# SimonZeng7108/efficientsam3

Measured on NVIDIA H100. Metric: encoder images/sec @1024^2 (EV-M student forward), higher is better.
Workload: dtype bf16

## Files before the change

### efficientsam3_b200/csrc/litemla_tc.cu

```cuda
#include "ptx.cuh"

namespace es3 {
namespace {
__device__ __forceinline__ void ldsm4t(uint32_t addr, uint32_t& r0, uint32_t& r1, uint32_t& r2, uint32_t& r3) {
  asm volatile("ldmatrix.sync.aligned.m8n8.x4.trans.shared.b16 {%0,%1,%2,%3}, [%4];"
               : "=r"(r0), "=r"(r1), "=r"(r2), "=r"(r3) : "r"(addr));
}
__device__ __forceinline__ void cpa16(uint32_t saddr, const void* g, bool valid) {
  const int sz = valid ? 16 : 0;
  asm volatile("cp.async.cg.shared.global [%0], [%1], 16, %2;" ::"r"(saddr), "l"(g), "r"(sz) : "memory");
}
__device__ __forceinline__ void cpa_wait_all() { asm volatile("cp.async.commit_group;\ncp.async.wait_group 0;" ::: "memory"); }
__device__ __forceinline__ uint32_t relu_bf16x2(uint32_t v) {
  uint32_t r;
  asm("max.bf16x2 %0, %1, %2;" : "=r"(r) : "r"(v), "r"(0u));
  return r;
}
}

constexpr int AG_TH = 16, AG_TW = 32, AG_IH = AG_TH + 4, AG_IW = AG_TW + 4, AG_PS = 48;
constexpr int AG_TILE_BYTES = AG_IH * AG_IW * AG_PS;

constexpr int AG2_SMEM = AG_TILE_BYTES + 25 * 16 * 2 + 16 * AG_PS;
__global__ void __launch_bounds__(256, 3) litemla_aggreg_dwpw_kernel(const bf16* ms_in, bf16* ms_out, long long ld,
                                                                  const bf16* __restrict__ wdw, const bf16* __restrict__ wpw,
                                                                  int H, int W, int tiles_x) {
  extern __shared__ __align__(16) uint8_t smem[];
  const uint32_t u_tile = static_cast<uint32_t>(__cvta_generic_to_shared(smem));
  const bf16* s_wd = reinterpret_cast<const bf16*>(smem + AG_TILE_BYTES);
  const uint32_t u_wp = u_tile + AG_TILE_BYTES + 25 * 16 * 2;
  const int tid = threadIdx.x, warp = tid >> 5, lane = tid & 31;
  const int tile = blockIdx.x, grp = blockIdx.y, b = blockIdx.z;
  const int oy0 = (tile / tiles_x) * AG_TH, ox0 = (tile % tiles_x) * AG_TW;

  const bf16* xb = ms_in + (long long)b * H * W * ld + grp * 16;
  for (int i = tid; i < AG_IH * AG_IW * 2; i += 256) {
    const int v = i & 1, p = i >> 1;
    const int iy = oy0 - 2 + p / AG_IW, ix = ox0 - 2 + p % AG_IW;
    const bool ok = iy >= 0 && iy < H && ix >= 0 && ix < W;
    cpa16(u_tile + p * AG_PS + v * 16, ok ? xb + ((long long)iy * W + ix) * ld + v * 8 : xb, ok);
  }
  if (tid < 50) cpa16(u_tile + AG_TILE_BYTES + tid * 16, wdw + (long long)grp * 400 + tid * 8, true);
  if (tid >= 64 && tid < 96) {
    const int i = tid - 64, n = i >> 1, v = i & 1;
    cpa16(u_wp + n * AG_PS + v * 16, wpw + ((long long)grp * 16 + n) * 16 + v * 8, true);
  }
  cpa_wait_all();
  __syncthreads();

  const int a_row = lane & 15, a_kh = lane >> 4;
  const int b_n = (lane & 7) + ((lane >> 4) << 3), b_kh = (lane >> 3) & 1;
  const int g = lane >> 2, t4 = lane & 3;
  const uint32_t dshift = (g & 1) ? 16u : 0u;
  const bool dvalid = (g >> 1) == t4;
  float acc[4][2][4];
#pragma unroll
  for (int m = 0; m < 4; ++m)
#pragma unroll
    for (int n = 0; n < 2; ++n) { acc[m][n][0] = acc[m][n][1] = acc[m][n][2] = acc[m][n][3] = 0.f; }

  const int xh = warp & 1, y0 = (warp >> 1) * 4;
#pragma unroll 1
  for (int kx = 0; kx < 5; ++kx) {
    uint32_t af[8][4];
#pragma unroll
    for (int r = 0; r < 8; ++r)
      ptx::ldsm_x4(u_tile + ((y0 + r) * AG_IW + xh * 16 + a_row + kx) * AG_PS + a_kh * 16, af[r][0], af[r][1], af[r][2], af[r][3]);
    uint32_t b_lo[5], b_hi[5];
#pragma unroll
    for (int ky = 0; ky < 5; ++ky) {
      const uint32_t w_lo = (uint32_t)__bfloat16_as_ushort(s_wd[(ky * 5 + kx) * 16 + g]);
      const uint32_t w_hi = (uint32_t)__bfloat16_as_ushort(s_wd[(ky * 5 + kx) * 16 + 8 + g]);
      b_lo[ky] = dvalid ? (w_lo << dshift) : 0u;
      b_hi[ky] = dvalid ? (w_hi << dshift) : 0u;
    }
#pragma unroll
    for (int m = 0; m < 4; ++m) {
#pragma unroll
      for (int kp = 0; kp < 2; ++kp) {
        const uint32_t a_lo[4] = {af[m + 2 * kp][0], af[m + 2 * kp][1], af[m + 2 * kp + 1][0], af[m + 2 * kp + 1][1]};
        const uint32_t a_hi[4] = {af[m + 2 * kp][2], af[m + 2 * kp][3], af[m + 2 * kp + 1][2], af[m + 2 * kp + 1][3]};
        ptx::mma_16816(acc[m][0], a_lo, b_lo[2 * kp], b_lo[2 * kp + 1]);
        ptx::mma_16816(acc[m][1], a_hi, b_hi[2 * kp], b_hi[2 * kp + 1]);
      }
      ptx::mma_1688(acc[m][0], af[m + 4][0], af[m + 4][1], b_lo[4]);
      ptx::mma_1688(acc[m][1], af[m + 4][2], af[m + 4][3], b_hi[4]);
    }
  }
  uint32_t p0, p1, p2, p3;
  ptx::ldsm_x4(u_wp + b_n * AG_PS + b_kh * 16, p0, p1, p2, p3);
  bf16* ob = ms_out + (long long)b * H * W * ld + grp * 16;
#pragma unroll
  for (int m = 0; m < 4; ++m) {
    const uint32_t pa[4] = {pack_bf16x2(acc[m][0][0], acc[m][0][1]), pack_bf16x2(acc[m][0][2], acc[m][0][3]),
                            pack_bf16x2(acc[m][1][0], acc[m][1][1]), pack_bf16x2(acc[m][1][2], acc[m][1][3])};
    float o[2][4] = {{0.f, 0.f, 0.f, 0.f}, {0.f, 0.f, 0.f, 0.f}};
    ptx::mma_16816(o[0], pa, p0, p1);
    ptx::mma_16816(o[1], pa, p2, p3);
    const int oy = oy0 + y0 + m;
    if (oy >= H) continue;
#pragma unroll
    for (int half = 0; half < 2; ++half) {
      const int ox = ox0 + xh * 16 + g + half * 8;
      if (ox >= W) continue;
      bf16* dst = ob + ((long long)oy * W + ox) * ld + t4 * 2;
      *reinterpret_cast<uint32_t*>(dst) = pack_bf16x2(o[0][half * 2], o[0][half * 2 + 1]);
      *reinterpret_cast<uint32_t*>(dst + 8) = pack_bf16x2(o[1][half * 2], o[1][half * 2 + 1]);
    }
  }
}

constexpr int KV_PX = 512, KV_RS = 80;

__global__ void __launch_bounds__(256) litemla_kv_tc_kernel(const bf16* __restrict__ ms, long long ld,
                                                            float* __restrict__ part, int HW) {
  __shared__ __align__(16) uint8_t s_kv[KV_PX * KV_RS];
  const uint32_t u = static_cast<uint32_t>(__cvta_generic_to_shared(s_kv));
  const int tid = threadIdx.x, warp = tid >> 5, lane = tid & 31;
  const int h = blockIdx.y, b = blockIdx.z, heads2 = gridDim.y, nchunk = gridDim.x;
  const int p_base = blockIdx.x * KV_PX;
  const bf16* src = ms + (long long)b * HW * ld + h * 48 + 16;
  for (int i = tid; i < KV_PX * 4; i += 256) {
    const int v = i & 3, pl = i >> 2;
    const bool ok = p_base + pl < HW;
    cpa16(u + pl * KV_RS + v * 16, ok ? src + (long long)(p_base + pl) * ld + v * 8 : src, ok);
  }
  cpa_wait_all();
  __syncthreads();

  const int g = lane >> 2, t4 = lane & 3;
  float acc[2][4], ones[2][4];
#pragma unroll
  for (int n = 0; n < 2; ++n) {
    acc[n][0] = acc[n][1] = acc[n][2] = acc[n][3] = 0.f;
    ones[n][0] = ones[n][1] = ones[n][2] = ones[n][3] = 0.f;
  }
  const uint32_t one2 = (g == 0) ? 0x3F803F80u : 0u;
  const uint32_t a_ones[4] = {one2, 0u, one2, 0u};
  const int av_p = (lane & 7) + ((lane >> 4) << 3), av_c = 32 + ((lane >> 3) & 1) * 16;
  const int bk_p = (lane & 7) + (((lane >> 3) & 1) << 3), bk_c = (lane >> 4) * 16;
#pragma unroll
  for (int ks = 0; ks < 4; ++ks) {
    const int p0 = warp * 64 + ks * 16;
    uint32_t af[4], b0, b1, b2, b3;
    ldsm4t(u + (p0 + av_p) * KV_RS + av_c, af[0], af[1], af[2], af[3]);
    ldsm4t(u + (p0 + bk_p) * KV_RS + bk_c, b0, b1, b2, b3);
    b0 = relu_bf16x2(b0); b1 = relu_bf16x2(b1); b2 = relu_bf16x2(b2); b3 = relu_bf16x2(b3);
    ptx::mma_16816(acc[0], af, b0, b1);
    ptx::mma_16816(acc[1], af, b2, b3);
    ptx::mma_16816(ones[0], a_ones, b0, b1);
    ptx::mma_16816(ones[1], a_ones, b2, b3);
  }
  __syncthreads();
  float* red = reinterpret_cast<float*>(s_kv);
  float* mine = red + warp * 17 * 16;
#pragma unroll
  for (int n = 0; n < 2; ++n) {
    const int j = n * 8 + t4 * 2;
    mine[g * 16 + j] = acc[n][0];
    mine[g * 16 + j + 1] = acc[n][1];
    mine[(g + 8) * 16 + j] = acc[n][2];
    mine[(g + 8) * 16 + j + 1] = acc[n][3];
    if (g == 0) {
      mine[16 * 16 + j] = ones[n][0];
      mine[16 * 16 + j + 1] = ones[n][1];
    }
  }
  __syncthreads();
  float* dst = part + (((long long)b * heads2 + h) * nchunk + blockIdx.x) * 17 * 16;
  for (int i = tid; i < 17 * 16; i += 256) {
    float s = 0.f;
#pragma unroll
    for (int w = 0; w < 8; ++w) s += red[w * 17 * 16 + i];
    dst[i] = s;
  }
}

__global__ void __launch_bounds__(128) litemla_apply_tc_kernel(const bf16* __restrict__ ms, long long ld,
                                                               const float* __restrict__ part, int nchunk,
                                                               bf16* __restrict__ att, long long ldo, int HW, float eps) {
  __shared__ float skv[17 * 16];
  const int tid = threadIdx.x, warp = tid >> 5, lane = tid & 31;
  const int h = blockIdx.y, b = blockIdx.z, heads2 = gridDim.y;
  const float* src = part + ((long long)b * heads2 + h) * nchunk * 17 * 16;
  for (int i = tid; i < 17 * 16; i += 128) {
    float a = 0.f;
    for (int c = 0; c < nchunk; ++c) a += src[c * 17 * 16 + i];
    skv[i] = a;
  }
  __syncthreads();
  const int g = lane >> 2, t4 = lane & 3;
  uint32_t bh[3][2], bl[3][2];
#pragma unroll
  for (int nt = 0; nt < 3; ++nt) {
    const int d = nt * 8 + g;
#pragma unroll
    for (int kh = 0; kh < 2; ++kh) {
      float v0 = 0.f, v1 = 0.f;
      if (d <= 16) { v0 = skv[d * 16 + kh * 8 + t4 * 2]; v1 = skv[d * 16 + kh * 8 + t4 * 2 + 1]; }
      const uint32_t hi = pack_bf16x2(v0, v1);
      const float2 hf = unpack_bf16x2(hi);
      bh[nt][kh] = hi;
      bl[nt][kh] = pack_bf16x2(v0 - hf.x, v1 - hf.y);
    }
  }
  const bf16* qb = ms + (long long)b * HW * ld + h * 48;
  bf16* ob = att + (long long)b * HW * ldo + h * 16;
#pragma unroll 1
  for (int mt = 0; mt < 4; ++mt) {
    const int p0 = blockIdx.x * 256 + warp * 64 + mt * 16;
    if (p0 >= HW) break;
    const int pa = p0 + g, pb = p0 + g + 8;
    uint32_t af[4] = {0u, 0u, 0u, 0u};
    if (pa < HW) {
      const uint32_t* q = reinterpret_cast<const uint32_t*>(qb + (long long)pa * ld);
      af[0] = relu_bf16x2(__ldg(q + t4));
      af[2] = relu_bf16x2(__ldg(q + 4 + t4));
    }
    if (pb < HW) {
      const uint32_t* q = reinterpret_cast<const uint32_t*>(qb + (long long)pb * ld);
      af[1] = relu_bf16x2(__ldg(q + t4));
      af[3] = relu_bf16x2(__ldg(q + 4 + t4));
    }
    float acc[3][4];
#pragma unroll
    for (int nt = 0; nt < 3; ++nt) {
      acc[nt][0] = acc[nt][1] = acc[nt][2] = acc[nt][3] = 0.f;
      ptx::mma_16816(acc[nt], af, bl[nt][0], bl[nt][1]);
      ptx::mma_16816(acc[nt], af, bh[nt][0], bh[nt][1]);
    }
    const float den_a = __shfl_sync(0xffffffffu, acc[2][0], g * 4);
    const float den_b = __shfl_sync(0xffffffffu, acc[2][2], g * 4);
    const float ia = 1.f / (den_a + eps), ib = 1.f / (den_b + eps);
    if (pa < HW) {
      uint32_t* o = reinterpret_cast<uint32_t*>(ob + (long long)pa * ldo);
      o[t4] = pack_bf16x2(acc[0][0] * ia, acc[0][1] * ia);
      o[4 + t4] = pack_bf16x2(acc[1][0] * ia, acc[1][1] * ia);
    }
    if (pb < HW) {
      uint32_t* o = reinterpret_cast<uint32_t*>(ob + (long long)pb * ldo);
      o[t4] = pack_bf16x2(acc[0][2] * ib, acc[0][3] * ib);
      o[4 + t4] = pack_bf16x2(acc[1][2] * ib, acc[1][3] * ib);
    }
  }
}

}

using namespace es3;

extern "C" int es3_litemla_aggreg_dwpw(void* ms, long long ld, const void* wdw, const void* wpw, int B, int H, int W, int C3,
                                       void* stream) {
  ES3_REQUIRE(C3 % 16 == 0 && ld % 8 == 0 && ld >= 2 * C3, "es3_litemla_aggreg_dwpw: bad C3=%d ld=%lld", C3, ld);
  static bool configured = false;
  if (!configured) {
    ES3_CHECK_CUDA(cudaFuncSetAttribute(litemla_aggreg_dwpw_kernel, cudaFuncAttributeMaxDynamicSharedMemorySize, AG2_SMEM));
    configured = true;
  }
  const int tiles_x = ceil_div(W, AG_TW), tiles_y = ceil_div(H, AG_TH);
  dim3 grid(tiles_x * tiles_y, C3 / 16, B);
  litemla_aggreg_dwpw_kernel<<<grid, 256, AG2_SMEM, (cudaStream_t)stream>>>((const bf16*)ms, (bf16*)ms + C3, ld, (const bf16*)wdw,
                                                                            (const bf16*)wpw, H, W, tiles_x);
  ES3_LAUNCH_CHECK("litemla_aggreg_dwpw_kernel");
  return 0;
}

extern "C" long long es3_litemla_ws_floats(int B, int HW, int heads2) {
  return (long long)B * heads2 * ceil_div(HW, KV_PX) * 17 * 16;
}

extern "C" int es3_litemla_attn_tc(const void* ms, long long ld, float* kv_ws, void* att, long long ldo, int B, int HW,
                                   int heads2, float eps, void* stream) {
  ES3_REQUIRE(ld >= 48 * heads2 && ld % 8 == 0 && ldo % 8 == 0, "es3_litemla_attn_tc: bad ld=%lld ldo=%lld heads2=%d", ld, ldo, heads2);
  cudaStream_t st = (cudaStream_t)stream;
  const int nchunk = ceil_div(HW, KV_PX);
  litemla_kv_tc_kernel<<<dim3(nchunk, heads2, B), 256, 0, st>>>((const bf16*)ms, ld, kv_ws, HW);
  ES3_LAUNCH_CHECK("litemla_kv_tc_kernel");
  litemla_apply_tc_kernel<<<dim3(ceil_div(HW, 256), heads2, B), 128, 0, st>>>((const bf16*)ms, ld, kv_ws, nchunk,
                                                                             (bf16*)att, ldo, HW, eps);
  ES3_LAUNCH_CHECK("litemla_apply_tc_kernel");
  return 0;
}
```

Measured before the change: 4031.

## Make LiteMLA kv/apply kernels persistent, multi-head, cp.async-pipelined, and reverse batch order

The kv and apply attention kernels become persistent-style, sized from SM occupancy. Each CTA handles several heads and several pixel chunks and streams them through a 3-stage cp.async ring, which hides load latency and cuts launch/tail overhead. The apply kernel now stages Q in shared memory and writes outputs through shared memory as coalesced 128-bit stores. The aggreg and apply kernels also walk the batch index in reverse, likely so they reuse the L2-resident data the previous kernel just touched. In exchange, dynamic shared memory and register use grow, and there is extra per-item synchronisation.

New measurement: 4074, median of 6. 1.1% higher.

```diff
diff --git a/efficientsam3_b200/csrc/litemla_tc.cu b/efficientsam3_b200/csrc/litemla_tc.cu
--- a/efficientsam3_b200/csrc/litemla_tc.cu
+++ b/efficientsam3_b200/csrc/litemla_tc.cu
@@ -11,10 +11,29 @@
   asm volatile("cp.async.cg.shared.global [%0], [%1], 16, %2;" ::"r"(saddr), "l"(g), "r"(sz) : "memory");
 }
 __device__ __forceinline__ void cpa_wait_all() { asm volatile("cp.async.commit_group;\ncp.async.wait_group 0;" ::: "memory"); }
+__device__ __forceinline__ void cpa_commit() { asm volatile("cp.async.commit_group;" ::: "memory"); }
+template <int N>
+__device__ __forceinline__ void cpa_wait() { asm volatile("cp.async.wait_group %0;" ::"n"(N) : "memory"); }
 __device__ __forceinline__ uint32_t relu_bf16x2(uint32_t v) {
   uint32_t r;
   asm("max.bf16x2 %0, %1, %2;" : "=r"(r) : "r"(v), "r"(0u));
   return r;
+}
+__device__ __forceinline__ void sts32(uint32_t addr, uint32_t v) { asm volatile("st.shared.b32 [%0], %1;" ::"r"(addr), "r"(v) : "memory"); }
+__device__ __forceinline__ uint4 lds128(uint32_t addr) {
+  uint4 v;
+  asm volatile("ld.shared.v4.b32 {%0,%1,%2,%3}, [%4];" : "=r"(v.x), "=r"(v.y), "=r"(v.z), "=r"(v.w) : "r"(addr) : "memory");
+  return v;
+}
+
+int sm_count() {
+  static int n = 0;
+  if (n == 0) {
+    int dev = 0;
+    ES3_CHECK_CUDA(cudaGetDevice(&dev));
+    ES3_CHECK_CUDA(cudaDeviceGetAttribute(&n, cudaDevAttrMultiProcessorCount, dev));
+  }
+  return n;
 }
 }
 
@@ -30,7 +49,7 @@
   const bf16* s_wd = reinterpret_cast<const bf16*>(smem + AG_TILE_BYTES);
   const uint32_t u_wp = u_tile + AG_TILE_BYTES + 25 * 16 * 2;
   const int tid = threadIdx.x, warp = tid >> 5, lane = tid & 31;
-  const int tile = blockIdx.x, grp = blockIdx.y, b = blockIdx.z;
+  const int tile = blockIdx.x, grp = blockIdx.y, b = gridDim.z - 1 - blockIdx.z;
   const int oy0 = (tile / tiles_x) * AG_TH, ox0 = (tile % tiles_x) * AG_TW;
 
   const bf16* xb = ms_in + (long long)b * H * W * ld + grp * 16;
@@ -110,139 +129,218 @@
   }
 }
 
-constexpr int KV_PX = 512, KV_RS = 80;
-
-__global__ void __launch_bounds__(256) litemla_kv_tc_kernel(const bf16* __restrict__ ms, long long ld,
-                                                            float* __restrict__ part, int HW) {
-  __shared__ __align__(16) uint8_t s_kv[KV_PX * KV_RS];
-  const uint32_t u = static_cast<uint32_t>(__cvta_generic_to_shared(s_kv));
+constexpr int KV_PX = 512, KV_NH = 2, KV_NS = 3;
+constexpr int KV_SPX = 128;
+constexpr int KV_RS = KV_NH * 96 + 16;
+constexpr int KV_STAGE = KV_SPX * KV_RS;
+constexpr int KV_SMEM = KV_NS * KV_STAGE + 8 * KV_NH * 17 * 16 * 4;
+
+__global__ void __launch_bounds__(256, 2) litemla_kv_tc_kernel(const bf16* __restrict__ ms, long long ld,
+                                                               float* __restrict__ part, int HW, int heads2, int nchunk, int cpc) {
+  extern __shared__ __align__(16) uint8_t smem[];
+  const uint32_t u = static_cast<uint32_t>(__cvta_generic_to_shared(smem));
+  float* red = reinterpret_cast<float*>(smem + KV_NS * KV_STAGE);
   const int tid = threadIdx.x, warp = tid >> 5, lane = tid & 31;
-  const int h = blockIdx.y, b = blockIdx.z, heads2 = gridDim.y, nchunk = gridDim.x;
-  const int p_base = blockIdx.x * KV_PX;
-  const bf16* src = ms + (long long)b * HW * ld + h * 48 + 16;
-  for (int i = tid; i < KV_PX * 4; i += 256) {
-    const int v = i & 3, pl = i >> 2;
-    const bool ok = p_base + pl < HW;
-    cpa16(u + pl * KV_RS + v * 16, ok ? src + (long long)(p_base + pl) * ld + v * 8 : src, ok);
-  }
-  cpa_wait_all();
-  __syncthreads();
+  const int h0 = blockIdx.y * KV_NH, b = blockIdx.z, nh = min(KV_NH, heads2 - h0);
+  const int c0 = blockIdx.x * cpc, nc = min(cpc, nchunk - c0), nitems = nc * 4;
+  const bf16* src = ms + (long long)b * HW * ld + h0 * 48;
+
+  auto load_item = [&](int k) {
+    const uint32_t us = u + (k % KV_NS) * KV_STAGE;
+    const int pbase = (c0 + (k >> 2)) * KV_PX + (k & 3) * 16;
+    for (int i = tid; i < KV_SPX * 6 * KV_NH; i += 256) {
+      const int c = i % (6 * KV_NH), r = i / (6 * KV_NH);
+      if (c >= 6 * nh || c % 6 < 2) continue;
+      const int p = pbase + (r >> 4) * 64 + (r & 15);
+      const bool ok = p < HW;
+      cpa16(us + r * KV_RS + c * 16, ok ? src + (long long)p * ld + c * 8 : src, ok);
+    }
+  };
+#pragma unroll
+  for (int s = 0; s < KV_NS - 1; ++s) {
+    if (s < nitems) load_item(s);
+    cpa_commit();
+  }
 
   const int g = lane >> 2, t4 = lane & 3;
-  float acc[2][4], ones[2][4];
-#pragma unroll
-  for (int n = 0; n < 2; ++n) {
-    acc[n][0] = acc[n][1] = acc[n][2] = acc[n][3] = 0.f;
-    ones[n][0] = ones[n][1] = ones[n][2] = ones[n][3] = 0.f;
-  }
   const uint32_t one2 = (g == 0) ? 0x3F803F80u : 0u;
   const uint32_t a_ones[4] = {one2, 0u, one2, 0u};
-  const int av_p = (lane & 7) + ((lane >> 4) << 3), av_c = 32 + ((lane >> 3) & 1) * 16;
-  const int bk_p = (lane & 7) + (((lane >> 3) & 1) << 3), bk_c = (lane >> 4) * 16;
-#pragma unroll
-  for (int ks = 0; ks < 4; ++ks) {
-    const int p0 = warp * 64 + ks * 16;
-    uint32_t af[4], b0, b1, b2, b3;
-    ldsm4t(u + (p0 + av_p) * KV_RS + av_c, af[0], af[1], af[2], af[3]);
-    ldsm4t(u + (p0 + bk_p) * KV_RS + bk_c, b0, b1, b2, b3);
-    b0 = relu_bf16x2(b0); b1 = relu_bf16x2(b1); b2 = relu_bf16x2(b2); b3 = relu_bf16x2(b3);
-    ptx::mma_16816(acc[0], af, b0, b1);
-    ptx::mma_16816(acc[1], af, b2, b3);
-    ptx::mma_16816(ones[0], a_ones, b0, b1);
-    ptx::mma_16816(ones[1], a_ones, b2, b3);
-  }
-  __syncthreads();
-  float* red = reinterpret_cast<float*>(s_kv);
-  float* mine = red + warp * 17 * 16;
-#pragma unroll
-  for (int n = 0; n < 2; ++n) {
-    const int j = n * 8 + t4 * 2;
-    mine[g * 16 + j] = acc[n][0];
-    mine[g * 16 + j + 1] = acc[n][1];
-    mine[(g + 8) * 16 + j] = acc[n][2];
-    mine[(g + 8) * 16 + j + 1] = acc[n][3];
-    if (g == 0) {
-      mine[16 * 16 + j] = ones[n][0];
-      mine[16 * 16 + j + 1] = ones[n][1];
-    }
-  }
-  __syncthreads();
-  float* dst = part + (((long long)b * heads2 + h) * nchunk + blockIdx.x) * 17 * 16;
-  for (int i = tid; i < 17 * 16; i += 256) {
-    float s = 0.f;
-#pragma unroll
-    for (int w = 0; w < 8; ++w) s += red[w * 17 * 16 + i];
-    dst[i] = s;
-  }
-}
-
-__global__ void __launch_bounds__(128) litemla_apply_tc_kernel(const bf16* __restrict__ ms, long long ld,
-                                                               const float* __restrict__ part, int nchunk,
-                                                               bf16* __restrict__ att, long long ldo, int HW, float eps) {
-  __shared__ float skv[17 * 16];
+  const int av_p = (lane & 7) + ((lane >> 4) << 3), av_c = 64 + ((lane >> 3) & 1) * 16;
+  const int bk_p = (lane & 7) + (((lane >> 3) & 1) << 3), bk_c = 32 + (lane >> 4) * 16;
+  float acc[KV_NH][2][4], ones[KV_NH][2][4];
+
+#pragma unroll 1
+  for (int k = 0; k < nitems; ++k) {
+    cpa_wait<KV_NS - 2>();
+    __syncthreads();
+    if (k + KV_NS - 1 < nitems) load_item(k + KV_NS - 1);
+    cpa_commit();
+    const int ks = k & 3;
+    if (ks == 0) {
+#pragma unroll
+      for (int j = 0; j < KV_NH; ++j)
+#pragma unroll
+        for (int n = 0; n < 2; ++n) {
+          acc[j][n][0] = acc[j][n][1] = acc[j][n][2] = acc[j][n][3] = 0.f;
+          ones[j][n][0] = ones[j][n][1] = ones[j][n][2] = ones[j][n][3] = 0.f;
+        }
+    }
+    const uint32_t us = u + (k % KV_NS) * KV_STAGE + warp * 16 * KV_RS;
+#pragma unroll
+    for (int j = 0; j < KV_NH; ++j) {
+      if (j >= nh) break;
+      uint32_t af[4], b0, b1, b2, b3;
+      ldsm4t(us + av_p * KV_RS + j * 96 + av_c, af[0], af[1], af[2], af[3]);
+      ldsm4t(us + bk_p * KV_RS + j * 96 + bk_c, b0, b1, b2, b3);
+      b0 = relu_bf16x2(b0); b1 = relu_bf16x2(b1); b2 = relu_bf16x2(b2); b3 = relu_bf16x2(b3);
+      ptx::mma_16816(acc[j][0], af, b0, b1);
+      ptx::mma_16816(acc[j][1], af, b2, b3);
+      ptx::mma_16816(ones[j][0], a_ones, b0, b1);
+      ptx::mma_16816(ones[j][1], a_ones, b2, b3);
+    }
+    if (ks != 3) continue;
+#pragma unroll
+    for (int j = 0; j < KV_NH; ++j) {
+      float* mine = red + (warp * KV_NH + j) * 17 * 16;
+#pragma unroll
+      for (int n = 0; n < 2; ++n) {
+        const int jj = n * 8 + t4 * 2;
+        mine[g * 16 + jj] = acc[j][n][0];
+        mine[g * 16 + jj + 1] = acc[j][n][1];
+        mine[(g + 8) * 16 + jj] = acc[j][n][2];
+        mine[(g + 8) * 16 + jj + 1] = acc[j][n][3];
+        if (g == 0) {
+          mine[16 * 16 + jj] = ones[j][n][0];
+          mine[16 * 16 + jj + 1] = ones[j][n][1];
+        }
+      }
+    }
+    __syncthreads();
+    const int chunk = c0 + (k >> 2);
+    for (int i = tid; i < nh * 17 * 16; i += 256) {
+      const int j = i / (17 * 16), e = i % (17 * 16);
+      float s = 0.f;
+#pragma unroll
+      for (int w = 0; w < 8; ++w) s += red[(w * KV_NH + j) * 17 * 16 + e];
+      part[(((long long)b * heads2 + h0 + j) * nchunk + chunk) * 17 * 16 + e] = s;
+    }
+  }
+  cpa_wait<0>();
+}
+
+constexpr int AP_NH = 4, AP_NS = 3;
+constexpr int AP_PX = 128;
+constexpr int AP_RS = AP_NH * 32 + 16;
+constexpr int AP_STAGE = AP_PX * AP_RS;
+constexpr int AP_SMEM = AP_NS * AP_STAGE + AP_NH * 17 * 16 * 4;
+
+__global__ void __launch_bounds__(256, 3) litemla_apply_tc_kernel(const bf16* __restrict__ ms, long long ld,
+                                                                  const float* __restrict__ part, int nchunk,
+                                                                  bf16* __restrict__ att, long long ldo, int HW, int heads2,
+                                                                  int spc, float eps) {
+  extern __shared__ __align__(16) uint8_t smem[];
+  const uint32_t u = static_cast<uint32_t>(__cvta_generic_to_shared(smem));
+  float* skv = reinterpret_cast<float*>(smem + AP_NS * AP_STAGE);
   const int tid = threadIdx.x, warp = tid >> 5, lane = tid & 31;
-  const int h = blockIdx.y, b = blockIdx.z, heads2 = gridDim.y;
-  const float* src = part + ((long long)b * heads2 + h) * nchunk * 17 * 16;
-  for (int i = tid; i < 17 * 16; i += 128) {
+  const int h0 = blockIdx.y * AP_NH, b = gridDim.z - 1 - blockIdx.z, nh = min(AP_NH, heads2 - h0);
+  const int s0 = blockIdx.x * spc, ns = min(spc, (HW + AP_PX - 1) / AP_PX - s0);
+  const bf16* qb = ms + (long long)b * HW * ld + h0 * 48;
+  bf16* ob = att + (long long)b * HW * ldo + h0 * 16;
+
+  auto load_stage = [&](int k) {
+    const uint32_t us = u + (k % AP_NS) * AP_STAGE;
+    const int pbase = (s0 + k) * AP_PX;
+    for (int i = tid; i < AP_PX * 2 * AP_NH; i += 256) {
+      const int c = i % (2 * AP_NH), r = i / (2 * AP_NH);
+      if (c >= 2 * nh) continue;
+      const bool ok = pbase + r < HW;
+      cpa16(us + r * AP_RS + c * 16, ok ? qb + (long long)(pbase + r) * ld + (c >> 1) * 48 + (c & 1) * 8 : qb, ok);
+    }
+  };
+#pragma unroll
+  for (int s = 0; s < AP_NS - 1; ++s) {
+    if (s < ns) load_stage(s);
+    cpa_commit();
+  }
+
+  const float* src = part + ((long long)b * heads2 + h0) * nchunk * 17 * 16;
+  for (int i = tid; i < nh * 17 * 16; i += 256) {
+    const int j = i / (17 * 16), e = i % (17 * 16);
+    const float* sj = src + (long long)j * nchunk * 17 * 16 + e;
     float a = 0.f;
-    for (int c = 0; c < nchunk; ++c) a += src[c * 17 * 16 + i];
+    for (int c = 0; c < nchunk; ++c) a += sj[c * 17 * 16];
     skv[i] = a;
   }
   __syncthreads();
   const int g = lane >> 2, t4 = lane & 3;
-  uint32_t bh[3][2], bl[3][2];
-#pragma unroll
-  for (int nt = 0; nt < 3; ++nt) {
-    const int d = nt * 8 + g;
-#pragma unroll
-    for (int kh = 0; kh < 2; ++kh) {
-      float v0 = 0.f, v1 = 0.f;
-      if (d <= 16) { v0 = skv[d * 16 + kh * 8 + t4 * 2]; v1 = skv[d * 16 + kh * 8 + t4 * 2 + 1]; }
-      const uint32_t hi = pack_bf16x2(v0, v1);
-      const float2 hf = unpack_bf16x2(hi);
-      bh[nt][kh] = hi;
-      bl[nt][kh] = pack_bf16x2(v0 - hf.x, v1 - hf.y);
-    }
-  }
-  const bf16* qb = ms + (long long)b * HW * ld + h * 48;
-  bf16* ob = att + (long long)b * HW * ldo + h * 16;
+  uint32_t bh[AP_NH][3][2], bl[AP_NH][3][2];
+#pragma unroll
+  for (int j = 0; j < AP_NH; ++j)
+#pragma unroll
+    for (int nt = 0; nt < 3; ++nt) {
+      const int d = nt * 8 + g;
+#pragma unroll
+      for (int kh = 0; kh < 2; ++kh) {
+        float v0 = 0.f, v1 = 0.f;
+        if (d <= 16 && j < nh) { v0 = skv[(j * 17 + d) * 16 + kh * 8 + t4 * 2]; v1 = skv[(j * 17 + d) * 16 + kh * 8 + t4 * 2 + 1]; }
+        const uint32_t hi = pack_bf16x2(v0, v1);
+        const float2 hf = unpack_bf16x2(hi);
+        bh[j][nt][kh] = hi;
+        bl[j][nt][kh] = pack_bf16x2(v0 - hf.x, v1 - hf.y);
+      }
+    }
+
 #pragma unroll 1
-  for (int mt = 0; mt < 4; ++mt) {
-    const int p0 = blockIdx.x * 256 + warp * 64 + mt * 16;
-    if (p0 >= HW) break;
-    const int pa = p0 + g, pb = p0 + g + 8;
-    uint32_t af[4] = {0u, 0u, 0u, 0u};
-    if (pa < HW) {
-      const uint32_t* q = reinterpret_cast<const uint32_t*>(qb + (long long)pa * ld);
-      af[0] = relu_bf16x2(__ldg(q + t4));
-      af[2] = relu_bf16x2(__ldg(q + 4 + t4));
-    }
-    if (pb < HW) {
-      const uint32_t* q = reinterpret_cast<const uint32_t*>(qb + (long long)pb * ld);
-      af[1] = relu_bf16x2(__ldg(q + t4));
-      af[3] = relu_bf16x2(__ldg(q + 4 + t4));
-    }
-    float acc[3][4];
-#pragma unroll
-    for (int nt = 0; nt < 3; ++nt) {
-      acc[nt][0] = acc[nt][1] = acc[nt][2] = acc[nt][3] = 0.f;
-      ptx::mma_16816(acc[nt], af, bl[nt][0], bl[nt][1]);
-      ptx::mma_16816(acc[nt], af, bh[nt][0], bh[nt][1]);
-    }
-    const float den_a = __shfl_sync(0xffffffffu, acc[2][0], g * 4);
-    const float den_b = __shfl_sync(0xffffffffu, acc[2][2], g * 4);
-    const float ia = 1.f / (den_a + eps), ib = 1.f / (den_b + eps);
-    if (pa < HW) {
-      uint32_t* o = reinterpret_cast<uint32_t*>(ob + (long long)pa * ldo);
-      o[t4] = pack_bf16x2(acc[0][0] * ia, acc[0][1] * ia);
-      o[4 + t4] = pack_bf16x2(acc[1][0] * ia, acc[1][1] * ia);
-    }
-    if (pb < HW) {
-      uint32_t* o = reinterpret_cast<uint32_t*>(ob + (long long)pb * ldo);
-      o[t4] = pack_bf16x2(acc[0][2] * ib, acc[0][3] * ib);
-      o[4 + t4] = pack_bf16x2(acc[1][2] * ib, acc[1][3] * ib);
-    }
-  }
+  for (int k = 0; k < ns; ++k) {
+    cpa_wait<AP_NS - 2>();
+    __syncthreads();
+    if (k + AP_NS - 1 < ns) load_stage(k + AP_NS - 1);
+    cpa_commit();
+    const uint32_t us = u + (k % AP_NS) * AP_STAGE;
+    const uint32_t uw = us + warp * 16 * AP_RS;
+#pragma unroll
+    for (int j = 0; j < AP_NH; ++j) {
+      if (j >= nh) break;
+      uint32_t af[4];
+      ptx::ldsm_x4(uw + (lane & 15) * AP_RS + j * 32 + (lane >> 4) * 16, af[0], af[1], af[2], af[3]);
+      af[0] = relu_bf16x2(af[0]); af[1] = relu_bf16x2(af[1]); af[2] = relu_bf16x2(af[2]); af[3] = relu_bf16x2(af[3]);
+      float acc[3][4];
+#pragma unroll
+      for (int nt = 0; nt < 3; ++nt) {
+        acc[nt][0] = acc[nt][1] = acc[nt][2] = acc[nt][3] = 0.f;
+        ptx::mma_16816(acc[nt], af, bl[j][nt][0], bl[j][nt][1]);
+        ptx::mma_16816(acc[nt], af, bh[j][nt][0], bh[j][nt][1]);
+      }
+      const float den_a = __shfl_sync(0xffffffffu, acc[2][0], g * 4);
+      const float den_b = __shfl_sync(0xffffffffu, acc[2][2], g * 4);
+      const float ia = 1.f / (den_a + eps), ib = 1.f / (den_b + eps);
+      __syncwarp();
+      const uint32_t oa = uw + g * AP_RS + j * 32 + t4 * 4, obb = oa + 8 * AP_RS;
+      sts32(oa, pack_bf16x2(acc[0][0] * ia, acc[0][1] * ia));
+      sts32(oa + 16, pack_bf16x2(acc[1][0] * ia, acc[1][1] * ia));
+      sts32(obb, pack_bf16x2(acc[0][2] * ib, acc[0][3] * ib));
+      sts32(obb + 16, pack_bf16x2(acc[1][2] * ib, acc[1][3] * ib));
+    }
+    __syncthreads();
+    const int pbase = (s0 + k) * AP_PX;
+    for (int i = tid; i < AP_PX * 2 * AP_NH; i += 256) {
+      const int c = i % (2 * AP_NH), r = i / (2 * AP_NH);
+      if (c >= 2 * nh || pbase + r >= HW) continue;
+      *reinterpret_cast<uint4*>(ob + (long long)(pbase + r) * ldo + c * 8) = lds128(us + r * AP_RS + c * 16);
+    }
+  }
+  cpa_wait<0>();
+}
+
+template <typename K>
+static int resident_ctas(K kern, int threads, int smem, bool& configured) {
+  if (!configured) {
+    ES3_CHECK_CUDA(cudaFuncSetAttribute(kern, cudaFuncAttributeMaxDynamicSharedMemorySize, smem));
+    configured = true;
+  }
+  int n = 0;
+  ES3_CHECK_CUDA(cudaOccupancyMaxActiveBlocksPerMultiprocessor(&n, kern, threads, smem));
+  return n > 0 ? n : 1;
 }
 
 }
@@ -273,11 +371,23 @@
                                    int heads2, float eps, void* stream) {
   ES3_REQUIRE(ld >= 48 * heads2 && ld % 8 == 0 && ldo % 8 == 0, "es3_litemla_attn_tc: bad ld=%lld ldo=%lld heads2=%d", ld, ldo, heads2);
   cudaStream_t st = (cudaStream_t)stream;
-  const int nchunk = ceil_div(HW, KV_PX);
-  litemla_kv_tc_kernel<<<dim3(nchunk, heads2, B), 256, 0, st>>>((const bf16*)ms, ld, kv_ws, HW);
+  static bool kv_configured = false, ap_configured = false;
+  static int kv_per_sm = 0, ap_per_sm = 0;
+  if (kv_per_sm == 0) kv_per_sm = resident_ctas(litemla_kv_tc_kernel, 256, KV_SMEM, kv_configured);
+  if (ap_per_sm == 0) ap_per_sm = resident_ctas(litemla_apply_tc_kernel, 256, AP_SMEM, ap_configured);
+  const int slots_kv = sm_count() * kv_per_sm, slots_ap = sm_count() * ap_per_sm;
+
+  const int nchunk = ceil_div(HW, KV_PX), kv_hb = ceil_div(heads2, KV_NH);
+  const int cpc = std::max(1, std::min(nchunk, ceil_div((long long)nchunk * kv_hb * B, slots_kv)));
+  litemla_kv_tc_kernel<<<dim3(ceil_div(nchunk, cpc), kv_hb, B), 256, KV_SMEM, st>>>((const bf16*)ms, ld, kv_ws, HW, heads2,
+                                                                                   nchunk, cpc);
   ES3_LAUNCH_CHECK("litemla_kv_tc_kernel");
-  litemla_apply_tc_kernel<<<dim3(ceil_div(HW, 256), heads2, B), 128, 0, st>>>((const bf16*)ms, ld, kv_ws, nchunk,
-                                                                             (bf16*)att, ldo, HW, eps);
+
+  const int nstage = ceil_div(HW, AP_PX), ap_hb = ceil_div(heads2, AP_NH);
+  const int want = std::max(1, std::min(nstage, slots_ap / std::max(1, ap_hb * B)));
+  const int spc = ceil_div(nstage, want);
+  litemla_apply_tc_kernel<<<dim3(ceil_div(nstage, spc), ap_hb, B), 256, AP_SMEM, st>>>((const bf16*)ms, ld, kv_ws, nchunk,
+                                                                                      (bf16*)att, ldo, HW, heads2, spc, eps);
   ES3_LAUNCH_CHECK("litemla_apply_tc_kernel");
   return 0;
 }
```
